# Kuldaen/Babylon.js-PathTracing-Renderer

Measured on AMD Instinct MI355X. Metric: Mpaths/s + achieved HBM GB/s, StanfordDragon 1080p 1spp, 1/2/4/8 MI355X, higher is better.
Workload: dtype f32

## Files before the change

### babylon.js-pathtracing-renderer_amd/csrc/pt_device.h

```cpp
#pragma once
#include <hip/hip_runtime.h>
#include <stdint.h>

#include "pt_args.h"
#include "pt_glsl.h"

namespace pt {
using namespace ptg;

constexpr float kINF = 1000000.0f;
constexpr float kTwoPi = 6.28318530717958648f;

enum { PROG_CORNELL = 3, PROG_GLTF = 4, PROG_HDRI = 5, PROG_SKY = 6, PROG_QUADRIC = 7, PROG_SKYMESH = 8 };
enum { PROG_TEX = 100, PROG_GLTF_TEX = 104, PROG_HDRI_TEX = 105, PROG_SKYMESH_TEX = 108 };
enum { PROG_PAIRS = 1000, PROG_TRAIL = 2000 };
template <int P> constexpr int kBase = P % PROG_PAIRS;
template <int P> constexpr int kScene = kBase<P> % PROG_TEX;
template <int P> constexpr bool kHasMesh = kScene<P> == PROG_GLTF || kScene<P> == PROG_HDRI || kScene<P> == PROG_SKYMESH;
template <int P> constexpr bool kIsGltf = kScene<P> == PROG_GLTF || kScene<P> == PROG_HDRI;
template <int P> constexpr bool kIsHdri = kScene<P> == PROG_HDRI;
template <int P> constexpr bool kHasTex = kBase<P> >= PROG_TEX;
template <int P> constexpr bool kIsSky = kScene<P> == PROG_SKY || kScene<P> == PROG_SKYMESH;
template <int P> constexpr bool kIsQuadric = P == PROG_QUADRIC;
template <int P> constexpr int kQuadId0 = kIsQuadric<P> ? 12 : 2;
template <int P> constexpr int kWalk = P / PROG_PAIRS;
template <int P> constexpr bool kPairs = P >= PROG_PAIRS;
template <int P> constexpr bool kTrail = kWalk<P> == WALK_TRAIL;
#define PT_FOR_EACH_PROG_REF(X)                                                                                           \
    X(PROG_CORNELL) X(PROG_SKY) X(PROG_QUADRIC) X(PROG_GLTF) X(PROG_GLTF_TEX) X(PROG_HDRI) X(PROG_HDRI_TEX)           \
    X(PROG_SKYMESH) X(PROG_SKYMESH_TEX)
#define PT_FOR_EACH_MESH_PROG(X, W)                                                                                       \
    X(W + PROG_GLTF) X(W + PROG_GLTF_TEX) X(W + PROG_HDRI) X(W + PROG_HDRI_TEX) X(W + PROG_SKYMESH) X(W + PROG_SKYMESH_TEX)
#define PT_FOR_EACH_PROG_PAIRS(X) PT_FOR_EACH_MESH_PROG(X, PROG_PAIRS)
#define PT_FOR_EACH_PROG_TRAIL(X) PT_FOR_EACH_MESH_PROG(X, PROG_TRAIL)
#define PT_FOR_EACH_PROG(X) PT_FOR_EACH_PROG_REF(X) PT_FOR_EACH_PROG_PAIRS(X) PT_FOR_EACH_PROG_TRAIL(X)

__host__ __device__ inline int resolveProgram(int prog, bool textured, int walk)
{
    if (prog != PROG_GLTF && prog != PROG_HDRI && prog != PROG_SKYMESH) return prog;
    return prog + (textured ? PROG_TEX : 0) + walk * PROG_PAIRS;
}
constexpr int kMinWavesTex = 4, kMinWavesPairs = 8, kMinWavesRef = 4;
template <int P> constexpr int kMinWaves = kHasTex<P> ? kMinWavesTex : kPairs<P> ? kMinWavesPairs : kMinWavesRef;
constexpr int kGoutLdsGltf = 0, kGoutLdsSky = 0;
template <int P> constexpr bool kPairs8 = kPairs<P> && !kHasTex<P>;
template <int P> constexpr int kGoutLdsOf = !kPairs8<P> ? 6 : kIsGltf<P> ? kGoutLdsGltf
                                          : kScene<P> == PROG_SKYMESH ? kGoutLdsSky : 6;
template <int P> constexpr int kStackLdsOf = kPairs8<P> ? (2 * kStackLdsPairs + 8 - kGoutLdsOf<P>) / 2 : kStackLds;
template <int P> constexpr int kRingOf = kHasTex<P> ? 14 : kPairs8<P> ? (2 * kStackLdsPairs + 8 - kGoutLdsOf<P>) / 2 : 6;
template <int P> constexpr bool kScratchOf = !kPairs8<P>;
template <int P> constexpr int kWalkSlotsOf = kTrail<P> ? kRingOf<P> : kStackLdsOf<P> + (kScratchOf<P> ? 1 : 0);

typedef float vf2 __attribute__((ext_vector_type(2)));
typedef __attribute__((address_space(3))) vf2 lds_float2;
typedef __attribute__((address_space(1))) vf2 glb_float2;

struct Path {
    uint32_t s0, s1;
    uint32_t bn;
    f3 ro, rd;
};
PT_D float unorm8(unsigned b);
PT_D float pathCounter(const Path& p) { return (float)((p.bn >> 16) & 0x7fu) - 1.0f; }
PT_D void setPathCounter(Path& p, float c) { p.bn = (p.bn & 0xff80ffffu) | ((unsigned)(c + 1.0f) << 16); }

PT_D float rng(Path& p)
{
    p.s0 += 1u; p.s1 += 1u;
    uint32_t qx = 1103515245u * ((p.s0 >> 1u) ^ p.s1);
    uint32_t qy = 1103515245u * ((p.s1 >> 1u) ^ p.s0);
    uint32_t n = 1103515245u * (qx ^ (qy >> 3u));
    return (float)n * (1.0f / 4294967296.0f);
}
PT_D float blueNoise_rand(Path& p)
{
    p.bn += 1u << 16;
    const unsigned channel = ((p.bn >> 16) - 1u) & 1u;
    return gfract(unorm8((p.bn >> (8u * channel)) & 255u));
}
PT_D float tentFilter(float x) { return (x < 0.5f) ? gsqrt(2.0f * x) - 1.0f : 1.0f - gsqrt(2.0f - (2.0f * x)); }
PT_D f3 onb_u(f3 nl)
{
    f3 a = (fabsf(nl.y) < 0.9f) ? mk(0.0f, 1.0f, 0.0f) : mk(1.0f, 0.0f, 0.0f);
    return normalize(cross(a, nl));
}
PT_D f3 cosWeightedDir(Path& p, f3 nl)
{
    float r = gsqrt(rng(p));
    float phi = rng(p) * kTwoPi;
    float sn, cs;
    gsincos(phi, sn, cs);
    float x = r * cs, y = r * sn;
    float z = gsqrt(1.0f - x * x - y * y);
    f3 U = onb_u(nl);
    f3 V = cross(nl, U);
    return normalize(U * x + V * y + nl * z);
}
PT_D f3 specularLobeDir(Path& p, f3 rdir, float roughness)
{
    roughness = gclamp(roughness, 0.0f, 1.0f);
    float exponent = gmix(7.0f, 0.0f, gsqrt(roughness));
    float cosTheta = gpow(rng(p), grcp(gexp(exponent) + 1.0f));
    float sinTheta = gsqrt(gmax(0.0f, 1.0f - cosTheta * cosTheta));
    float phi = rng(p) * kTwoPi;
    float sn, cs;
    gsincos(phi, sn, cs);
    f3 U = onb_u(rdir);
    f3 V = cross(rdir, U);
    f3 lobe = (U * cs) * sinTheta + (V * sn) * sinTheta + rdir * cosTheta;
    return normalize(mix3(rdir, lobe, roughness));
}
PT_D float fresnel(f3 rdir, f3 n, float etai, float etat, float& ratioIoR)
{
    float temp = etai;
    float cosi = gclamp(dot(rdir, n), -1.0f, 1.0f);
    if (cosi > 0.0f) { etai = etat; etat = temp; }
    ratioIoR = etai / etat;
    float sint = ratioIoR * gsqrt(1.0f - (cosi * cosi));
    if (sint >= 1.0f) return 1.0f;
    float cost = gsqrt(1.0f - (sint * sint));
    cosi = fabsf(cosi);
    float Rs = ((etat * cosi) - (etai * cost)) / ((etat * cosi) + (etai * cost));
    float Rp = ((etai * cosi) - (etat * cost)) / ((etai * cosi) + (etat * cost));
    return gclamp(((Rs * Rs) + (Rp * Rp)) * 0.5f, 0.0f, 1.0f);
}
PT_D f3 sampleQuadLight(Path& p, const TraceArgs& a, f3 x, f3 nl, float& weight)
{
    const QuadArg& L = a.light;
    f3 q;
    q.x = gmix(L.v0.x, L.v2.x, gclamp(rng(p), 0.1f, 0.9f));
    q.y = gmix(L.v0.y, L.v2.y, gclamp(rng(p), 0.1f, 0.9f));
    q.z = gmix(L.v0.z, L.v2.z, gclamp(rng(p), 0.1f, 0.9f));
    f3 d = q - x;
    float d2 = dot(d, d);
    float cos_a_max = gsqrt(1.0f - gclamp(a.light_r2 / d2, 0.0f, 1.0f));
    d = normalize(d);
    float dotNl = gmax(0.0f, dot(nl, d));
    float w = 2.0f * (1.0f - cos_a_max) * gmax(0.0f, -dot(d, L.normal)) * dotNl;
    weight = gclamp(w, 0.0f, 1.0f);
    return d;
}

PT_D float unitSphere(f3 ro, f3 rd, f3& n)
{
    float a = dot(rd, rd);
    float b = 2.0f * dot(rd, ro);
    float c = dot(ro, ro) - 1.0f;
    float invA = grcp(a);
    b *= invA;
    c *= invA;
    float nh = -b * 0.5f;
    float u2 = nh * nh - c;
    float u;
    if (u2 < 0.0f) { nh = 0.0f; u = 0.0f; } else u = gsqrt(u2);
    float t0 = nh - u, t1 = nh + u;
    float t = t0 > 0.0f ? t0 : t1 > 0.0f ? t1 : kINF;
    if (t != kINF) { f3 h = ro + rd * t; n = mk(2.0f * h.x, 2.0f * h.y, 2.0f * h.z); }
    return t;
}
PT_D bool recipNegative(float x) { return (x < 0.0f && x != -__builtin_inff()) || (x == 0.0f && __builtin_signbit(x)); }

PT_D float quadTriangle(const TriArg& T, f3 ro, f3 rd)
{
    f3 pv = cross(rd, T.e2);
    const float dd = dot(T.e1, pv);
    if (recipNegative(dd)) return kINF;
    float det = grcp(dd);
    f3 tv = ro - T.v0;
    float u = dot(tv, pv) * det;
    if (u < 0.0f || u > 1.0f) return kINF;
    f3 qv = cross(tv, T.e1);
    float v = dot(rd, qv) * det;
    float t = dot(T.e2, qv) * det;
    return (u < 0.0f || u > 1.0f || v < 0.0f || u + v > 1.0f || t <= 0.0f) ? kINF : t;
}
PT_D float box(f3 mn, f3 mx, f3 ro, f3 inv)
{
    f3 nr = (mn - ro) * inv;
    f3 fr = (mx - ro) * inv;
    float t0 = gmax(gmax(gmin(nr.x, fr.x), gmin(nr.y, fr.y)), gmin(nr.z, fr.z));
    float t1 = gmin(gmin(gmax(nr.x, fr.x), gmax(nr.y, fr.y)), gmax(nr.z, fr.z));
    return gmax(t0, 0.0f) > t1 ? kINF : t0;
}
PT_D float vmax0(float a) { float r; asm("v_max_f32 %0, 0, %1" : "=v"(r) : "v"(a)); return r; }
PT_D float boxFast(f3 mn, f3 mx, f3 ro, f3 inv)
{
    float t0, t1, a0, a1, a2, b0, b1, b2;
    asm("v_sub_f32 %2, %8, %14\n\t"
        "v_sub_f32 %3, %9, %15\n\t"
        "v_sub_f32 %4, %10, %16\n\t"
        "v_sub_f32 %5, %11, %14\n\t"
        "v_sub_f32 %6, %12, %15\n\t"
        "v_sub_f32 %7, %13, %16\n\t"
        "v_mul_f32 %2, %2, %17\n\t"
        "v_mul_f32 %3, %3, %18\n\t"
        "v_mul_f32 %4, %4, %19\n\t"
        "v_mul_f32 %5, %5, %17\n\t"
        "v_mul_f32 %6, %6, %18\n\t"
        "v_mul_f32 %7, %7, %19\n\t"
        "v_min_f32 %0, %2, %5\n\t"
        "v_max_f32 %2, %2, %5\n\t"
        "v_min_f32 %1, %3, %6\n\t"
        "v_max_f32 %3, %3, %6\n\t"
        "v_min_f32 %5, %4, %7\n\t"
// ... 394 lines not shown
```

### babylon.js-pathtracing-renderer_amd/csrc/pt_program.h

```cpp
#pragma once
#include <hip/hip_runtime.h>
#include <stdint.h>

#include "pt_args.h"
#include "pt_device.h"
#include "pt_glsl.h"
#include "pt_quadric.h"

namespace pt {

struct Hit {
    float t;
    f3 normal, color;
    float u, v;
    int type;
    int id;
};

struct Cnt {
    unsigned seg, node, leaf, hit, tap, ovf, hdr;
#ifdef PT_SECPROF
    unsigned long long* sec;
    unsigned lane_steps;
    unsigned sget, sget_slab, sput, sput_slab;
    unsigned bounce;
#endif
};
#ifdef PT_SECPROF
#define PT_SEC(cnt, k)                                                                        \
    do {                                                                                      \
        const unsigned long long now_ = clock64();                                            \
        const int ln_ = __lane_id();                                                          \
        if ((cnt).sec && ln_ == __builtin_amdgcn_readfirstlane(ln_)) {                \
            (cnt).sec[k] += now_ - (cnt).sec[8]; (cnt).sec[8] = now_;                         \
        }                                                                                     \
    } while (0)
#else
#define PT_SEC(cnt, k) do {} while (0)
#endif

struct GOut {
    static constexpr bool kColById = false;
    f3 nrm, col;
    float id, sharp;
    PT_D void clear() { nrm = mk(0, 0, 0); col = mk(0, 0, 0); id = 0.0f; sharp = 0.0f; }
    PT_D void pinCol(f3) {}
    PT_D void setNrm(f3 v) { nrm = v; }
    PT_D void setCol(f3 v) { col = v; }
    PT_D void setId(float v) { id = v; }
    PT_D void setSharp(float v) { sharp = v; }
};
typedef __attribute__((address_space(3))) float lds_float;
typedef __attribute__((address_space(1))) float glb_float;
template <int LS, int NF = 6>
struct GOutLds {
    static constexpr bool kColById = NF <= 3;
    lds_float* p;
    unsigned slot;
    glb_float* gx;
    unsigned gi, gs;
    uint32_t* bn;
    PT_D unsigned at(int f) const
    {
        unsigned i = gi;
        asm volatile("" : "+v"(i));
        return i + (unsigned)(f - NF) * gs;
    }
    PT_D void put(int f, float v)
    {
        if (f < NF) p[f * LS + slot] = v;
        else gx[at(f)] = v;
    }
    PT_D float get(int f) const
    {
        if (f < NF) return p[f * LS + slot];
        return ((*bn >> (f < 3 ? 23 : 31)) & 1u) ? gx[at(f)] : 0.0f;
    }
    PT_D void clear()
    {
        for (int f = 0; f < NF; f++) p[f * LS + slot] = 0.0f;
        *bn &= 0x007fffffu;
    }
    PT_D void setNrm(f3 v)
    {
        put(0, v.x); put(1, v.y); put(2, v.z);
        if (NF < 3 || kColById) *bn |= 1u << 23;
    }
    PT_D void setCol(f3 v)
    {
        if (kColById) return;
        put(3, v.x); put(4, v.y); put(5, v.z);
        if (NF < 6) *bn |= 1u << 31;
    }
    PT_D void pinCol(f3 v)
    {
        if (!kColById) return;
        put(3, v.x); put(4, v.y); put(5, v.z);
        *bn |= 1u << 31;
    }
    PT_D void setId(float v) { *bn = (*bn & ~(31u << 26)) | (((unsigned)(int)v & 31u) << 26); }
    PT_D void setSharp(float v)
    {
        const unsigned code = v == 1.01f ? 1u : v == -1.0f ? 2u : 0u;
        *bn = (*bn & ~(3u << 24)) | (code << 24);
    }
    PT_D float sharp() const
    {
        const unsigned code = (*bn >> 24) & 3u;
        return code == 1u ? 1.01f : code == 2u ? -1.0f : 0.0f;
    }
    PT_D float id() const { return (float)((*bn >> 26) & 31u); }
    template <class F>
    PT_D GOut load(F colOfId) const
    {
        GOut g;
        g.nrm = mk(get(0), get(1), get(2)); g.id = id(); g.sharp = sharp();
        if (!kColById) g.col = mk(get(3), get(4), get(5));
        else if (!((*bn >> 23) & 1u)) g.col = mk(0.0f, 0.0f, 0.0f);
        else g.col = ((*bn >> 31) & 1u) ? mk(get(3), get(4), get(5)) : colOfId(g.id);
        return g;
    }
};

struct PState {
    f3 mask;
    float roughness;
    int diffuseCount, hitType, bounce;
    bool coat, specular, sampleLight;
};

template <class G>
PT_D void pathBegin(PState& s, G& g)
{
    s.mask = mk(1, 1, 1);
    s.roughness = 0.0f;
    s.diffuseCount = 0; s.hitType = -100; s.bounce = 0;
    s.coat = false; s.specular = true; s.sampleLight = false;
    g.clear();
}

PT_D float rayleighPhase(float cosTheta) { return 0.05968310365946075f * (1.0f + (cosTheta * cosTheta)); }
PT_HD float hgPhase(float cosTheta, float g)
{
    float g2 = g * g;
    float inverse = grcp(gpow(gmax(0.0f, 1.0f - 2.0f * g * cosTheta + g2), 1.5f));
    return 0.07957747154594767f * ((1.0f - g2) * inverse);
}
PT_D f3 pow3(f3 v, float e) { return mk(gpow(v.x, e), gpow(v.y, e), gpow(v.z, e)); }
PT_D f3 skyColor(const SkyArgs& k, f3 rayDir)
{
    const f3 vd = normalize(rayDir);
    const float cosViewSunAngle = dot(vd, k.sun);
    const float zenithAngle = gacos(gmax(0.0f, dot(mk(0.0f, 1.0f, 0.0f), vd)));
    const float inverse =
        grcp(gcos(zenithAngle) + 0.15f * gpow(93.885f - ((zenithAngle * 180.0f) / 3.14159265358979323f), -1.253f));
    const float rl = 8400.0f * inverse, ml = 1250.0f * inverse;
    const f3 e = k.rayleigh * rl + k.mie * ml;
    const f3 Fex = mk(gexp(-e.x), gexp(-e.y), gexp(-e.z));
    const f3 betaR = k.rayleigh * rayleighPhase(cosViewSunAngle * 0.5f + 0.5f);
    const f3 betaM = k.mie * hgPhase(cosViewSunAngle, 0.76f);
    const f3 q = (betaR + betaM) / k.rm;
    f3 Lin = pow3((q * k.sunE) * (mk(1.0f, 1.0f, 1.0f) - Fex), 1.5f);
    const f3 m = pow3((q * k.sunE) * Fex, 1.0f / 2.0f);
    Lin = Lin * mk(gmix(1.0f, m.x, k.fade), gmix(1.0f, m.y, k.fade), gmix(1.0f, m.z, k.fade));
    f3 L0 = mk(0.1f, 0.1f, 0.1f) * Fex;
    const float sundisk = gsmoothstep(0.9998f, 0.9998f + 0.00002f, cosViewSunAngle);
    L0 = L0 + (Fex * k.sunE19000) * sundisk;
    const f3 tex = (Lin + L0) * 0.04f + mk(0.0f, 0.0003f, 0.00075f);
    return pow3(tex, k.retExp);
}

template <int PROG>
PT_D int meshObjectId(const TraceArgs& a) { return kQuadId0<PROG> + a.nquads; }

template <int PROG>
PT_D void objectMaterial(const TraceArgs& a, int id, f3& color, int& type)
{
    constexpr int q0 = kQuadId0<PROG>;
    if (kIsQuadric<PROG> && id >= 0 && id < q0) {
        const float cr[12] = { 1.0f, 0.0f, 1.0f, 1.0f, 1.0f, 0.5f, 0.0f, 0.0f, 0.2f, 0.0f, 1.0f, 0.5f };
        const float cg[12] = { 0.0f, 1.0f, 1.0f, 0.0f, 0.1f, 1.0f, 0.4f, 0.0f, 0.0f, 1.0f, 0.3f, 0.0f };
        const float cb[12] = { 0.0f, 0.0f, 0.0f, 1.0f, 0.0f, 0.0f, 1.0f, 1.0f, 1.0f, 0.5f, 0.0f, 1.0f };
        color = mk(cr[id], cg[id], cb[id]);
        type = a.shape_mat;
    } else if (!kIsQuadric<PROG> && id >= 0 && id < 2) {
        color = a.sph[id].color; type = a.sph[id].type;
    } else if (id >= q0 && id < q0 + a.nquads) {
        color = a.qcolor[id - q0]; type = a.qtype[id - q0];
    } else if (kHasMesh<PROG> && id == meshObjectId<PROG>(a)) {
        color = mk(1.0f, 1.0f, 1.0f); type = a.uses_albedo ? PBR_MATERIAL : a.model_mat;
    }
}

template <int PROG>
PT_D void analyticNearest(const TraceArgs& a, f3 rayO, f3 rayD, Hit& h, f3& sn)
{
    constexpr int q0 = kQuadId0<PROG>;
    h.t = kINF;
    h.type = -100;
    h.id = -1;
    sn = mk(0, 0, 0);
    if (kIsQuadric<PROG>) {
#pragma unroll 1
        for (int s = 0; s < 12; s++) {
            f3 n = mk(0, 0, 0);
            float d = quadricShape(s, mul(a.shape_inv[s], rayO, 1.0f), mul(a.shape_inv[s], rayD, 0.0f), a.shape_k, n);
            if (d < h.t) { h.t = d; h.id = s; sn = n; }
        }
    } else {
#pragma unroll 1
        for (int s = 0; s < 2; s++) {
            const SphereArg& S = a.sph[s];
            f3 n;
            float d = unitSphere(mul(S.inv, rayO, 1.0f), mul(S.inv, rayD, 0.0f), n);
            if (d < h.t) { h.t = d; h.id = s; sn = n; }
        }
    }
// ... 224 lines not shown
```

### babylon.js-pathtracing-renderer_amd/csrc/pt_trace.h

```cpp
#pragma once
#include <hip/hip_runtime.h>
#include <stdint.h>

#include "pt_args.h"
#include "pt_device.h"
#include "pt_glsl.h"
#include "pt_program.h"
#ifdef PT_SECPROF
#define PT_SECPROF_ON 1
#else
#define PT_SECPROF_ON 0
#endif

using namespace ptg;

namespace pt {

template <int LS, int NL, bool SCRATCH>
struct MegaStack {
    lds_float2* lds;
    unsigned slot;
    glb_float2* slab;
    unsigned deep;
    unsigned stride;
#ifdef PT_SECPROF
    mutable unsigned n_get = 0, n_get_slab = 0, n_put = 0, n_put_slab = 0;
#define PT_SLABCOUNT(x) x
#else
#define PT_SLABCOUNT(x)
#endif
    PT_D float2 pop(int si, float2 sentinel) const
    {
        PT_SLABCOUNT(n_get++; if (si >= NL) n_get_slab++;)
        vf2 e = lds[(unsigned)min(si, NL - 1) * LS + slot];
        if (si >= NL) {
            const vf2 s = { sentinel.x, sentinel.y };
            e = si < kStackLevels ? slab[(unsigned)(si - NL) * stride + deep] : s;
        }
        return make_float2(e.x, e.y);
    }
    PT_D bool push(int si, float2 e)
    {
        const vf2 v = { e.x, e.y };
        PT_SLABCOUNT(n_put++; if (si >= NL) n_put_slab++;)
        if (SCRATCH) lds[(unsigned)min(si, NL) * LS + slot] = v;
        else if (si < NL) lds[(unsigned)si * LS + slot] = v;
        if (si >= NL) {
            if (si >= kStackLevels) return false;
            slab[(unsigned)(si - NL) * stride + deep] = v;
        }
        return true;
    }
};

template <int PROG, bool COUNT>
PT_D void meshHit(const TraceArgs& a, float triID, float triU, float triV, Hit& h, Cnt& cnt)
{
    float4 v2 = fetch32(a.tri, a.tri_texels, triID + 2.0f), v3 = fetch32(a.tri, a.tri_texels, triID + 3.0f),
           v4 = fetch32(a.tri, a.tri_texels, triID + 4.0f), v5 = fetch32(a.tri, a.tri_texels, triID + 5.0f);
    if (COUNT) cnt.hit++;
    float triW = 1.0f - triU - triV;
    f3 nn = normalize(mk(v2.y, v2.z, v2.w) * triW + mk(v3.x, v3.y, v3.z) * triU + mk(v3.w, v4.x, v4.y) * triV);
    h.u = triW * v4.z + triU * v5.x + triV * v5.z;
    h.v = triW * v4.w + triU * v5.y + triV * v5.w;
    if (kHasTex<PROG> && a.uses_bump) {
        f3 S = onb_u(nn);
        f3 T = cross(nn, S);
        f3 N = normalize(nn);
        if (dot(cross(S, T), N) < 0.0f) { S = S * -1.0f; T = T * -1.0f; }
        float tx[4];
        texBilinear(a.bump, h.u, h.v, tx);
        if (COUNT) cnt.tap += 4;
        f3 mN = normalize(mk(tx[0] * 2.0f - 1.0f, tx[1] * 2.0f - 1.0f, tx[2] * 2.0f - 1.0f));
        mN.x *= 1.0f; mN.y *= 1.0f;
        nn = normalize(S * mN.x + T * mN.y + N * mN.z);
    }
    h.normal = normalize(mul3t(a.model, nn));
    h.type = a.uses_albedo ? PBR_MATERIAL : a.model_mat;
    h.color = mk(1.0f, 1.0f, 1.0f);
    h.id = meshObjectId<PROG>(a);
}

template <int PROG, bool COUNT, int LS>
PT_D void sceneIntersect(const TraceArgs& a, f3 rayO, f3 rayD, Hit& h, float2* lds, unsigned lane_slot,
                         unsigned deep, Cnt& cnt, bool firstHit)
{
    const bool anyHit = !COUNT && firstHit;
    if (COUNT) cnt.seg++;
    f3 sn;
    PT_SEC(cnt, 4);
    analyticNearest<PROG>(a, rayO, rayD, h, sn);
    PT_SEC(cnt, 1);
    if (!kHasMesh<PROG>) { analyticAttributes<PROG>(a, h, sn); PT_SEC(cnt, 3); return; }

    f3 O = mul(a.model, rayO, 1.0f), D = mul(a.model, rayD, 0.0f);
    f3 inv = mk(grcp(D.x), grcp(D.y), grcp(D.z));
    const bool dbl = (!a.uses_albedo && a.model_mat == TRANSPARENT);
    BvhResult br = { 0.0f, 0.0f, 0.0f, false, 1u, 0u, 0u };
    MegaStack<LS, kStackLdsOf<PROG>, kScratchOf<PROG>> st{ (lds_float2*)lds, lane_slot, (glb_float2*)a.spill, deep, a.spill_stride };
    if (kPairs<PROG>) {
        const float* rb = a.bvh_root_box;
        const float rootT = box(mk(rb[0], rb[1], rb[2]), mk(rb[3], rb[4], rb[5]), O, inv);
        auto walk = [&]() {
            if (kTrail<PROG>) bvhWalkTrail<kRingOf<PROG>>(a, O, D, inv, dbl, rootT, h.t, (lds_float2*)lds, LS, lane_slot, br);
            else bvhWalkPairs(a, O, D, inv, dbl, rootT, h.t, st, br, anyHit);
        };
#ifdef PT_SECPROF
        if (cnt.sec) {
            const int ln_ = __lane_id();
            if (ln_ == __builtin_amdgcn_readfirstlane(ln_)) cnt.sec[9] = 0;
            walk();
            atomicMax(&cnt.sec[9], (unsigned long long)br.steps);
            cnt.lane_steps += br.steps;
            if (ln_ == __builtin_amdgcn_readfirstlane(ln_)) cnt.sec[10] += cnt.sec[9];
        } else
#endif
        walk();
    } else {
        float4 c0 = fetch32(a.aabb, a.aabb_texels, 0.0f), c1 = fetch32(a.aabb, a.aabb_texels, 1.0f);
        const float rootT = box(mk(c0.y, c0.z, c0.w), mk(c1.y, c1.z, c1.w), O, inv);
        bvhWalkRef(a, O, D, inv, dbl, c0, c1, rootT, h.t, st, br);
    }
    if (COUNT) { cnt.node += br.nodes; cnt.leaf += br.leaves; cnt.ovf += br.ovf; }
#ifdef PT_SECPROF
    if (COUNT) { cnt.sget += st.n_get; cnt.sget_slab += st.n_get_slab + br.restarts; cnt.sput += st.n_put; cnt.sput_slab += st.n_put_slab; }
    br.ws.flush(a.walk_stat, cnt.bounce++);
#endif
    PT_SEC(cnt, 2);
    if (br.lookup && anyHit) {
        h.normal = mk(0.0f, 0.0f, 1.0f);
        h.type = a.uses_albedo ? PBR_MATERIAL : a.model_mat;
        h.color = mk(1.0f, 1.0f, 1.0f);
        h.id = meshObjectId<PROG>(a);
    } else if (br.lookup) meshHit<PROG, COUNT>(a, br.triID, br.triU, br.triV, h, cnt);
    else analyticAttributes<PROG>(a, h, sn);
    PT_SEC(cnt, 3);
}

template <int PROG, bool COUNT, int LS, class G>
PT_D bool bounceStep(const TraceArgs& a, Path& p, PState& s, G& g, f3& accum, float2* lds, unsigned lane_slot,
                     unsigned deep, Cnt& cnt)
{
    Hit h;
    const bool lastOk = !kHasTex<PROG> && !a.uses_albedo &&
                        (a.model_mat == DIFFUSE || a.model_mat == METAL || a.model_mat == TRANSPARENT);
    sceneIntersect<PROG, COUNT, LS>(a, p.ro, p.rd, h, lds, lane_slot, deep, cnt, s.sampleLight || (s.bounce == 5 && lastOk));
    return shadeStep<PROG, COUNT, G>(a, p, s, g, accum, h, cnt);
}

PT_D void contStore(const TraceArgs& a, unsigned slot, const Path& p, const PState& s)
{
    const unsigned bits = ((unsigned)s.diffuseCount & 0xffu) | (((unsigned)s.hitType & 0xffu) << 8) |
                          (((unsigned)s.bounce & 0xffu) << 16) | (s.coat ? 1u << 24 : 0u) |
                          (s.specular ? 1u << 25 : 0u) | (s.sampleLight ? 1u << 26 : 0u);
    float4* r = a.cont_rec + 4ull * slot;
    r[0] = make_float4(p.ro.x, p.ro.y, p.ro.z, p.rd.x);
    r[1] = make_float4(p.rd.y, p.rd.z, s.mask.x, s.mask.y);
    r[2] = make_float4(s.mask.z, s.roughness, __uint_as_float(p.s0), __uint_as_float(p.s1));
    r[3] = make_float4(__uint_as_float(p.bn), __uint_as_float(bits), 0.0f, 0.0f);
}
PT_D void contLoad(const TraceArgs& a, unsigned slot, Path& p, PState& s)
{
    const float4* r = a.cont_rec + 4ull * slot;
    const float4 r0 = r[0], r1 = r[1], r2 = r[2], r3 = r[3];
    p.ro = mk(r0.x, r0.y, r0.z); p.rd = mk(r0.w, r1.x, r1.y);
    s.mask = mk(r1.z, r1.w, r2.x); s.roughness = r2.y;
    p.s0 = __float_as_uint(r2.z); p.s1 = __float_as_uint(r2.w); p.bn = __float_as_uint(r3.x);
    const unsigned bits = __float_as_uint(r3.y);
    s.diffuseCount = (int)(bits & 0xffu);
    s.hitType = (int)(signed char)((bits >> 8) & 0xffu);
    s.bounce = (int)((bits >> 16) & 0xffu);
    s.coat = (bits >> 24) & 1u; s.specular = (bits >> 25) & 1u; s.sampleLight = (bits >> 26) & 1u;
}
struct GBits {
    static constexpr bool kColById = false;
    uint32_t* bn;
    PT_D void clear() {}
    PT_D void pinCol(f3) {}
    PT_D void setNrm(f3) {}
    PT_D void setCol(f3) {}
    PT_D void setId(float) {}
    PT_D float id() const { return 0.0f; }
    PT_D void setSharp(float v)
    {
        const unsigned code = v == 1.01f ? 1u : v == -1.0f ? 2u : 0u;
        *bn = (*bn & ~(3u << 24)) | (code << 24);
    }
    PT_D float sharp() const
    {
        const unsigned code = (*bn >> 24) & 3u;
        return code == 1u ? 1.01f : code == 2u ? -1.0f : 0.0f;
    }
};

PT_D void contRank(const TraceArgs& a, int slot, const Path& p, const PState& s, bool inside)
{
    unsigned key = 0u;
    if (inside) {
        const float* rb = a.bvh_root_box;
        const f3 o = mul(a.model, p.ro, 1.0f);
        const unsigned gb = a.cont_grid_bits;
        const int top = (1 << gb) - 1;
        const unsigned cx = (unsigned)min(top, max(0, (int)((o.x - rb[0]) * a.cont_cell[0])));
        const unsigned cy = (unsigned)min(top, max(0, (int)((o.y - rb[1]) * a.cont_cell[1])));
        const unsigned cz = (unsigned)min(top, max(0, (int)((o.z - rb[2]) * a.cont_cell[2])));
        auto spread = [](unsigned v) { return (v & 1u) | ((v & 2u) << 2) | ((v & 4u) << 4); };
        const unsigned cell = spread(cx) | (spread(cy) << 1) | (spread(cz) << 2);
        const unsigned oct = (p.rd.x < 0.0f ? 1u : 0u) | (p.rd.y < 0.0f ? 2u : 0u) | (p.rd.z < 0.0f ? 4u : 0u);
        const unsigned lt = s.sampleLight ? 1u : 0u;
        key = (lt << (3u + 3u * gb)) | (cell << 3) | oct;
    }
    unsigned long long todo = __ballot(inside), peers = 0ull;
    while (todo) {
        const int lead = __ffsll((long long)todo) - 1;
        const unsigned k = __shfl(key, lead, 64);
        const bool mine = inside && key == k;
        const unsigned long long m = __ballot(mine);
        if (mine) peers = m;
        todo &= ~m;
    }
    const int leader = inside ? __ffsll((long long)peers) - 1 : (int)__lane_id();
    unsigned base = 0u;
    if (inside && (int)__lane_id() == leader) base = atomicAdd(&a.cont_bins[key], (unsigned)__popcll(peers));
    base = __shfl(base, leader, 64);
    if (inside) {
        a.cont_key[slot] = (unsigned short)key;
        a.cont_rank[slot] = base + (unsigned)__popcll(peers & ((1ull << __lane_id()) - 1ull));
    }
}

template <int PROG, bool COUNT, int LS, bool CONT, class G>
PT_D f3 radiance(const TraceArgs& a, Path& p, G& g, float2* lds, unsigned lane_slot, unsigned deep, Cnt& cnt,
                 bool inside, int& slot)
{
    PState s;
    pathBegin(s, g);
    f3 accum = mk(0, 0, 0);
#pragma unroll 1
    while (bounceStep<PROG, COUNT, LS, G>(a, p, s, g, accum, lds, lane_slot, deep, cnt)) {
        if (CONT && (unsigned)s.bounce >= a.cont_bounce && (unsigned)__popcll(__ballot(1)) <= a.cont_lanes) {
            const unsigned long long st = __ballot(inside);
            const int lead = __ffsll((long long)__ballot(1)) - 1;
            unsigned base = 0;
            if (__lane_id() == lead && st) base = atomicAdd(a.cont_count, (unsigned)__popcll(st));
            base = __shfl(base, lead, 64);
            if (inside) {
                slot = (int)(base + (unsigned)__popcll(st & ((1ull << __lane_id()) - 1ull)));
                contStore(a, (unsigned)slot, p, s);
            }
            if (a.cont_bins) contRank(a, slot, p, s, inside);
            break;
        }
    }
    return max3s(accum, 0.0f);
}

PT_D void radianceOut(const TraceArgs& a, long long pi, f3 r, float sharp, bool edge)
{
    float ca = 0.0f;
    if (edge) sharp = 1.01f;
    if (sharp == 1.01f) ca = 1.01f;
    if (sharp == -1.0f) ca = -1.0f;
    typedef float nt4 __attribute__((ext_vector_type(4)));
    const nt4 o = { r.x, r.y, r.z, ca };
    __builtin_nontemporal_store(o, (nt4*)&a.rad[pi]);
}

PT_D void featureOut(const TraceArgs& a, long long pi, const GOut& g)
{
    typedef float nt4 __attribute__((ext_vector_type(4)));
    const nt4 n = { g.nrm.x, g.nrm.y, g.nrm.z, g.id };
    const nt4 c = { g.col.x, g.col.y, g.col.z, 0.0f };
    __builtin_nontemporal_store(n, (nt4*)&a.feat0[pi]);
    __builtin_nontemporal_store(c, (nt4*)&a.feat1[pi]);
}

PT_D float xorq(float v, int m) { return __shfl_xor(v, m, 64); }

constexpr int kCostBuckets = 128;

constexpr int kTraceBlock = 64;
constexpr int kTraceSub = 4;

struct TracePlace {
    int px, py, part;
    unsigned costIdx;
};
PT_D bool tracePlace(const TraceArgs& a, int lane, TracePlace& pl)
{
    int wave, part = -1;
    const unsigned tiles_x = gridDim.x / 4u, ntiles = a.ntiles;
    const unsigned K = (a.order && a.split) ? *a.split : 0u;
    const unsigned L = blockIdx.y * gridDim.x + blockIdx.x;
    unsigned slot;
    constexpr unsigned kPer = 4u * kSplitParts;
    if (L < kPer * K) {
        const unsigned g = L / (8u * kPer), r = L % (8u * kPer);
        slot = g * 8u + (r & 7u);
        wave = (int)((r >> 3) / kSplitParts);
        part = (int)((r >> 3) % kSplitParts);
    } else {
        const unsigned L2 = L - kPer * K;
        if (L2 >= 4u * (ntiles - K)) return false;
        const unsigned g = L2 >> 5, r = L2 & 31u;
        const unsigned T = min(8u, ntiles - K - g * 8u);
        slot = K + g * 8u + r % T;
        wave = (int)(r / T);
    }
    unsigned rank = slot;
    if (a.order_zig && slot >= K) {
        const unsigned j = slot - K, m = ntiles - K, g = j >> 3, t = (g >> 1) * 8u + (j & 7u);
        rank = K + ((g & 1u) ? m - 1u - t : t);
    }
    const unsigned tile = a.order ? a.order[rank] : slot;
    const int tx = (int)(tile % tiles_x);
    const unsigned bY = tile / tiles_x;
    int lx, ly;
    if (part < 0) { lx = (lane & 1) | ((lane >> 1) & 6); ly = ((lane >> 1) & 1) | ((lane >> 3) & 6); }
    else {
        lx = (part & 1) * 4 + ((lane & 1) | ((lane >> 1) & 2));
        ly = (part >> 1) * 4 + (((lane >> 1) & 1) | ((lane >> 2) & 2));
    }
    const int band = (int)bY * a.num_parts + a.part;
    pl.px = tx * kTile + (wave & 1) * 8 + lx;
    pl.py = band * kTile + (wave >> 1) * 8 + ly;
    pl.part = part;
    pl.costIdx = tile * 4u + (unsigned)wave;
    return true;
}

template <int PROG, bool COUNT, bool CONT, bool FEAT = false>
__global__ __launch_bounds__(kTraceBlock, kMinWaves<PROG>) void pt_trace(TraceArgs a)
{
    static_assert(!CONT || (kHasMesh<PROG> && !COUNT), "late-bounce compaction: mesh programs, timed kernels");
    static_assert(!FEAT || !COUNT, "feature staging: a variant of the timed kernels");
    __shared__ float2 lds_stack[kWalkSlotsOf<PROG> * kTraceBlock + (kGoutLdsOf<PROG> * kTraceBlock + 1) / 2];
    float* const lds_gout = (float*)(lds_stack + kWalkSlotsOf<PROG> * kTraceBlock);
    const unsigned tid = threadIdx.x;
    const int lane = tid & 63;
    const unsigned long long t_start = clock64();
#ifdef PT_SECPROF
    const unsigned long long w0_ = wall_clock64();
#endif
    TracePlace pl;
    if (!tracePlace(a, lane, pl)) return;
    const int px = pl.px, py = pl.py;
    const unsigned deep = (blockIdx.y * gridDim.x + blockIdx.x) * kTraceBlock + tid;

    const bool active = px < ((a.width + 1) & ~1) && py < ((a.height + 1) & ~1) && (pl.part < 0 || lane < (int)(64u / kSplitParts));
    Cnt cnt = { 0, 0, 0, 0, 0, 0, 0 };
#ifdef PT_SECPROF
    __shared__ unsigned long long lds_sec[16];
    if (tid < 16) lds_sec[tid] = tid == 8 ? clock64() : 0ull;
    cnt.sec = lds_sec;
    cnt.lane_steps = 0;
    cnt.sget = cnt.sget_slab = cnt.sput = cnt.sput_slab = 0;
    cnt.bounce = 0;
#endif
    glb_float* const gx = kGoutLdsOf<PROG> < 6
        ? (glb_float*)(a.spill + (size_t)(kStackLevels - kStackLdsMin) * a.spill_stride)
        : nullptr;
    Path p;
    p.bn = 0u;
    GOutLds<kTraceBlock, kGoutLdsOf<PROG>> gl{ (lds_float*)lds_gout, tid, gx, deep, a.spill_stride, &p.bn };
    gl.clear();
    f3 r = mk(0, 0, 0);
    int slot = -1;
    if (active) {
        cameraRay(a, px, py, p);
        PT_SEC(cnt, 0);
        r = radiance<PROG, COUNT, kTraceBlock, CONT>(a, p, gl, lds_stack, tid, deep, cnt, px < a.width && py < a.height, slot);
    }
    PT_SEC(cnt, 4);
    const GOut g = gl.load([&](float id) {
        f3 c = mk(0.0f, 0.0f, 0.0f);
        int t;
        objectMaterial<PROG>(a, (int)id, c, t);
        return c;
    });

    const bool xodd = lane & 1, yodd = lane & 2;
    auto ddx = [&](float v) { float o = xorq(v, 1); return xodd ? v - o : o - v; };
    auto ddy = [&](float v) { float o = xorq(v, 2); return yodd ? v - o : o - v; };
    float dNx = fabsf(ddx(g.nrm.x)) + fabsf(ddy(g.nrm.x));
    float dNy = fabsf(ddx(g.nrm.y)) + fabsf(ddy(g.nrm.y));
    float dNz = fabsf(ddx(g.nrm.z)) + fabsf(ddy(g.nrm.z));
    float normalDiff = gsmoothstep(0.2f, 0.6f, dNx) + gsmoothstep(0.2f, 0.6f, dNy) + gsmoothstep(0.2f, 0.6f, dNz);
    float dObj = fabsf(ddx(g.id)) > 0.0f ? 1.0f : 0.0f;
    dObj += fabsf(ddy(g.id)) > 0.0f ? 1.0f : 0.0f;
    float objectDiff = gsmoothstep(0.0f, 0.5f, dObj);
    f3 dcx = mk(ddx(g.col.x), ddx(g.col.y), ddx(g.col.z));
    f3 dcy = mk(ddy(g.col.x), ddy(g.col.y), ddy(g.col.z));
    float dCol = length(dcx) > 0.0f ? 1.0f : 0.0f;
    dCol += length(dcy) > 0.0f ? 1.0f : 0.0f;
    float colorDiff = gsmoothstep(0.0f, 0.5f, dCol);

#ifdef PT_SECPROF
    if (!COUNT && a.wave_log) {
        atomicMax(&lds_sec[11], (unsigned long long)cnt.lane_steps);
        if (tid == 0) {
            const unsigned L = blockIdx.y * gridDim.x + blockIdx.x;
            unsigned long long* wl = a.wave_log + (size_t)kWaveLogSlots * L;
            wl[0] = w0_;
            wl[1] = wall_clock64();
            wl[2] = lds_sec[10];
            wl[3] = lds_sec[11];
            for (int k = 0; k < 8; k++) wl[4 + k] = lds_sec[k];
            wl[12] = __smid();
        }
    }
    if (COUNT && active) {
        atomicAdd(&a.counters[3], (unsigned long long)cnt.sget_slab);
        atomicAdd(&a.counters[4], (unsigned long long)cnt.node);
        atomicAdd(&a.counters[5], (unsigned long long)cnt.leaf);
        atomicAdd(&a.counters[6], 1ull);
    }
#endif
    if (COUNT && active && !PT_SECPROF_ON) {
        unsigned long long* C = a.counters;
        atomicAdd(&C[C_PATHS], 1ull);
        atomicAdd(&C[C_SEGMENTS], (unsigned long long)cnt.seg);
        atomicAdd(&C[C_NODE], (unsigned long long)cnt.node);
        atomicAdd(&C[C_LEAF], (unsigned long long)cnt.leaf);
        atomicAdd(&C[C_HIT], (unsigned long long)cnt.hit);
        atomicAdd(&C[C_RGBA8], (unsigned long long)(cnt.tap + 1));
        atomicAdd(&C[C_OVERFLOW], (unsigned long long)cnt.ovf);
        atomicAdd(&C[C_HDR], (unsigned long long)cnt.hdr);
    }
    if (a.cost && lane == 0) {
        const unsigned long long dur = min(clock64() - t_start, 0xffffffffull);
        a.cost[pl.costIdx] = (unsigned)((dur + (unsigned long long)a.cost[pl.costIdx]) >> 1);
    }
    if (!active || px >= a.width || py >= a.height) return;
    const bool edge = colorDiff >= 1.0f || normalDiff >= 1.0f || objectDiff >= 1.0f;
    const long long pi = (long long)py * a.width + px;
    if (FEAT || (COUNT && a.feat0)) featureOut(a, pi, g);
    if (CONT && slot >= 0) {
        a.cont_aux[slot] = (unsigned)pi | (edge ? 0x80000000u : 0u);
        return;
    }
    radianceOut(a, pi, r, g.sharp, edge);
}

template <int PROG>
__global__ __launch_bounds__(kTraceBlock, kMinWaves<PROG>) void pt_cont(TraceArgs a)
{
    __shared__ float2 lds_stack[kWalkSlotsOf<PROG> * kTraceBlock];
    const unsigned lane = threadIdx.x;
    const unsigned n = a.cont_count[0];
    unsigned* const head = a.cont_count + 1;
    bool more = true;
    const unsigned deep = blockIdx.x * kTraceBlock + lane;
    const unsigned long long below = (1ull << lane) - 1ull;
    Cnt cnt = { 0, 0, 0, 0, 0, 0, 0 };
    Path p;
    p.bn = 0u;
    PState s;
    GBits g{ &p.bn };
    f3 accum = mk(0, 0, 0);
    unsigned slot = 0;
    bool alive = false;
    for (;;) {
        const unsigned long long dead = __ballot(!alive);
        const unsigned ndead = (unsigned)__popcll(dead);
        if (more && (ndead >= a.cont_refill || ndead == 64u)) {
            unsigned base = 0;
            if (lane == 0) base = atomicAdd(head, ndead);
            base = __shfl(base, 0, 64);
            if (base + ndead >= n) more = false;
            if (!alive) {
                const unsigned q = base + (unsigned)__popcll(dead & below);
                if (q < n) {
                    slot = a.cont_perm ? a.cont_perm[q] : q;
                    contLoad(a, slot, p, s);
                    accum = mk(0, 0, 0);
                    alive = true;
                }
            }
        }
        if (__ballot(alive) == 0ull) {
            if (!more) break;
            continue;
        }
        if (alive && !bounceStep<PROG, false, kTraceBlock>(a, p, s, g, accum, lds_stack, lane, deep, cnt)) {
            const unsigned aux = a.cont_aux[slot];
            radianceOut(a, (long long)(aux & 0x7fffffffu), max3s(accum, 0.0f), g.sharp(), (aux >> 31) != 0u);
            alive = false;
        }
    }
}

template <int PROG, bool COUNT>
__global__ __launch_bounds__(kBlock, kMinWaves<PROG>) void pt_persist(TraceArgs a, WfBufs w, int tiles_x,
                                                                       unsigned n_wave_tiles, unsigned per_wave,
                                                                       unsigned refill)
{
    __shared__ float2 lds_stack[kWalkSlotsOf<PROG> * kBlock];
    const unsigned tid = threadIdx.x;
    const unsigned lane = tid & 63u, wave = tid >> 6;
    const unsigned long long below = (1ull << lane) - 1ull;
    const unsigned wid = blockIdx.x * (kBlock / 64) + wave;
    unsigned next = wid * per_wave * 64u;
    const unsigned end = min(next + per_wave * 64u, n_wave_tiles * 64u);
    const unsigned deep = blockIdx.x * kBlock + tid;
    Cnt cnt = { 0, 0, 0, 0, 0, 0, 0 };
    unsigned paths = 0;
    Path p;
    PState s;
    GOut g;
    f3 accum = mk(0, 0, 0);
    unsigned pix = 0;
    bool alive = false;
    for (;;) {
        const unsigned long long dead = __ballot(!alive);
        const unsigned ndead = (unsigned)__popcll(dead);
        if (next < end && (ndead >= refill || ndead == 64u)) {
            if (!alive) {
                const unsigned q = next + (unsigned)__popcll(dead & below);
                if (q < end) {
                    const unsigned L = q >> 6, l = q & 63u;
                    const unsigned per_band = (unsigned)tiles_x * 4u;
                    const unsigned bl = L / per_band, rem = L - bl * per_band;
                    const unsigned tx = rem >> 2, sub = rem & 3u;
                    const int band = (int)bl * a.num_parts + a.part;
                    const int lx = (int)((l & 1u) | ((l >> 1) & 6u)), ly = (int)(((l >> 1) & 1u) | ((l >> 3) & 6u));
                    const int px = (int)tx * kTile + (int)(sub & 1u) * 8 + lx;
                    const int py = band * kTile + (int)(sub >> 1) * 8 + ly;
                    if (px < w.wq && py < w.hq) {
                        cameraRay(a, px, py, p);
                        pathBegin(s, g);
                        accum = mk(0, 0, 0);
                        pix = (unsigned)py * (unsigned)w.wq + (unsigned)px;
                        alive = true;
                        if (COUNT) paths++;
                    }
                }
            }
            next += ndead;
        }
        if (__ballot(alive) == 0ull) {
            if (next >= end) break;
            continue;
        }
        if (alive && !bounceStep<PROG, COUNT, kBlock>(a, p, s, g, accum, lds_stack, tid, deep, cnt)) {
            const f3 r = max3s(accum, 0.0f);
            w.gb0[pix] = make_float4(g.nrm.x, g.nrm.y, g.nrm.z, g.id);
            w.gb1[pix] = make_float4(g.col.x, g.col.y, g.col.z, g.sharp);
            w.rad[pix] = make_float4(r.x, r.y, r.z, 0.0f);
            alive = false;
        }
    }
    if (COUNT) {
        unsigned long long* C = a.counters;
        if (paths) atomicAdd(&C[C_PATHS], (unsigned long long)paths);
        atomicAdd(&C[C_SEGMENTS], (unsigned long long)cnt.seg);
        atomicAdd(&C[C_NODE], (unsigned long long)cnt.node);
        atomicAdd(&C[C_LEAF], (unsigned long long)cnt.leaf);
        atomicAdd(&C[C_HIT], (unsigned long long)cnt.hit);
        atomicAdd(&C[C_RGBA8], (unsigned long long)(cnt.tap + paths));
        atomicAdd(&C[C_OVERFLOW], (unsigned long long)cnt.ovf);
        atomicAdd(&C[C_HDR], (unsigned long long)cnt.hdr);
    }
}

}
```

Measured before the change: 3225.

## Recompute lane-derived indices and pack path state to cut live VGPRs across traversal

For the pairs BVH programs, the kernel stops keeping per-lane values live through BVH traversal. Spill and gout addresses now use a wave-uniform base plus the lane id recomputed with mbcnt. Pixel coordinates and the inside test are rebuilt after tracing, path state flags are packed into one register across sceneIntersect, and the sphere normal is recomputed after traversal. The continuation kernel keeps only mask, roughness and packed bits between steps. The aim is lower register pressure and higher occupancy in the traversal loop, at the cost of extra ALU work to recompute and unpack these values.

```diff
diff --git a/babylon.js-pathtracing-renderer_amd/csrc/pt_device.h b/babylon.js-pathtracing-renderer_amd/csrc/pt_device.h
--- a/babylon.js-pathtracing-renderer_amd/csrc/pt_device.h
+++ b/babylon.js-pathtracing-renderer_amd/csrc/pt_device.h
@@ -50,6 +50,14 @@
 template <int P> constexpr int kRingOf = kHasTex<P> ? 14 : kPairs8<P> ? (2 * kStackLdsPairs + 8 - kGoutLdsOf<P>) / 2 : 6;
 template <int P> constexpr bool kScratchOf = !kPairs8<P>;
 template <int P> constexpr int kWalkSlotsOf = kTrail<P> ? kRingOf<P> : kStackLdsOf<P> + (kScratchOf<P> ? 1 : 0);
+
+template <int P> constexpr bool kWaveBaseOf = kPairs8<P>;
+PT_D unsigned laneNow()
+{
+    unsigned l;
+    asm volatile("v_mbcnt_lo_u32_b32 %0, -1, 0\n\tv_mbcnt_hi_u32_b32 %0, -1, %0" : "=v"(l));
+    return l;
+}
 
 typedef float vf2 __attribute__((ext_vector_type(2)));
 typedef __attribute__((address_space(3))) vf2 lds_float2;
diff --git a/babylon.js-pathtracing-renderer_amd/csrc/pt_pathstate.h b/babylon.js-pathtracing-renderer_amd/csrc/pt_pathstate.h
--- /dev/null
+++ b/babylon.js-pathtracing-renderer_amd/csrc/pt_pathstate.h
@@ -0,0 +1,22 @@
+#pragma once
+#include <cstdint>
+
+namespace pt {
+
+struct PathBits {
+    int diffuseCount, hitType, bounce;
+    bool coat, specular, sampleLight;
+};
+
+constexpr uint32_t pathBitsPack(int diffuseCount, int hitType, int bounce, bool coat, bool specular, bool sampleLight)
+{
+    return ((uint32_t)diffuseCount & 0xffu) | (((uint32_t)hitType & 0xffu) << 8) | (((uint32_t)bounce & 0xffu) << 16) |
+           (coat ? 1u << 24 : 0u) | (specular ? 1u << 25 : 0u) | (sampleLight ? 1u << 26 : 0u);
+}
+constexpr PathBits pathBitsUnpack(uint32_t bits)
+{
+    return PathBits{ (int)(bits & 0xffu), (int)(((bits >> 8) & 0xffu) ^ 0x80u) - 0x80, (int)((bits >> 16) & 0xffu),
+                     ((bits >> 24) & 1u) != 0u, ((bits >> 25) & 1u) != 0u, ((bits >> 26) & 1u) != 0u };
+}
+
+}
diff --git a/babylon.js-pathtracing-renderer_amd/csrc/pt_program.h b/babylon.js-pathtracing-renderer_amd/csrc/pt_program.h
--- a/babylon.js-pathtracing-renderer_amd/csrc/pt_program.h
+++ b/babylon.js-pathtracing-renderer_amd/csrc/pt_program.h
@@ -52,7 +52,7 @@
 };
 typedef __attribute__((address_space(3))) float lds_float;
 typedef __attribute__((address_space(1))) float glb_float;
-template <int LS, int NF = 6>
+template <int LS, int NF = 6, bool BASE = false>
 struct GOutLds {
     static constexpr bool kColById = NF <= 3;
     lds_float* p;
@@ -62,7 +62,7 @@
     uint32_t* bn;
     PT_D unsigned at(int f) const
     {
-        unsigned i = gi;
+        unsigned i = BASE ? gi + laneNow() : gi;
         asm volatile("" : "+v"(i));
         return i + (unsigned)(f - NF) * gs;
     }
diff --git a/babylon.js-pathtracing-renderer_amd/csrc/pt_trace.h b/babylon.js-pathtracing-renderer_amd/csrc/pt_trace.h
--- a/babylon.js-pathtracing-renderer_amd/csrc/pt_trace.h
+++ b/babylon.js-pathtracing-renderer_amd/csrc/pt_trace.h
@@ -5,6 +5,7 @@
 #include "pt_args.h"
 #include "pt_device.h"
 #include "pt_glsl.h"
+#include "pt_pathstate.h"
 #include "pt_program.h"
 #ifdef PT_SECPROF
 #define PT_SECPROF_ON 1
@@ -16,13 +17,14 @@
 
 namespace pt {
 
-template <int LS, int NL, bool SCRATCH>
+template <int LS, int NL, bool SCRATCH, bool BASE>
 struct MegaStack {
     lds_float2* lds;
     unsigned slot;
     glb_float2* slab;
     unsigned deep;
     unsigned stride;
+    PT_D unsigned at() const { return BASE ? deep + laneNow() : deep; }
 #ifdef PT_SECPROF
     mutable unsigned n_get = 0, n_get_slab = 0, n_put = 0, n_put_slab = 0;
 #define PT_SLABCOUNT(x) x
@@ -35,7 +37,7 @@
         vf2 e = lds[(unsigned)min(si, NL - 1) * LS + slot];
         if (si >= NL) {
             const vf2 s = { sentinel.x, sentinel.y };
-            e = si < kStackLevels ? slab[(unsigned)(si - NL) * stride + deep] : s;
+            e = si < kStackLevels ? slab[(unsigned)(si - NL) * stride + at()] : s;
         }
         return make_float2(e.x, e.y);
     }
@@ -47,7 +49,7 @@
         else if (si < NL) lds[(unsigned)si * LS + slot] = v;
         if (si >= NL) {
             if (si >= kStackLevels) return false;
-            slab[(unsigned)(si - NL) * stride + deep] = v;
+            slab[(unsigned)(si - NL) * stride + at()] = v;
         }
         return true;
     }
@@ -81,7 +83,22 @@
     h.id = meshObjectId<PROG>(a);
 }
 
-template <int PROG, bool COUNT, int LS>
+template <int PROG> constexpr bool kNormalAfter = kHasMesh<PROG> && !kIsQuadric<PROG>;
+PT_D f3 sphereNormal(const TraceArgs& a, f3 rayO, f3 rayD, const Hit& h)
+{
+    f3 n = mk(0, 0, 0);
+#pragma unroll 1
+    for (int s = 0; s < 2; s++) {
+        if (h.id != s) continue;
+        const SphereArg& S = a.sph[s];
+        const f3 ro = mul(S.inv, rayO, 1.0f), rd = mul(S.inv, rayD, 0.0f);
+        const f3 x = ro + rd * h.t;
+        n = mk(2.0f * x.x, 2.0f * x.y, 2.0f * x.z);
+    }
+    return n;
+}
+
+template <int PROG, bool COUNT, int LS, bool SLIM>
 PT_D void sceneIntersect(const TraceArgs& a, f3 rayO, f3 rayD, Hit& h, float2* lds, unsigned lane_slot,
                          unsigned deep, Cnt& cnt, bool firstHit)
 {
@@ -97,7 +114,7 @@
     f3 inv = mk(grcp(D.x), grcp(D.y), grcp(D.z));
     const bool dbl = (!a.uses_albedo && a.model_mat == TRANSPARENT);
     BvhResult br = { 0.0f, 0.0f, 0.0f, false, 1u, 0u, 0u };
-    MegaStack<LS, kStackLdsOf<PROG>, kScratchOf<PROG>> st{ (lds_float2*)lds, lane_slot, (glb_float2*)a.spill, deep, a.spill_stride };
+    MegaStack<LS, kStackLdsOf<PROG>, kScratchOf<PROG>, SLIM> st{ (lds_float2*)lds, lane_slot, (glb_float2*)a.spill, deep, a.spill_stride };
     if (kPairs<PROG>) {
         const float* rb = a.bvh_root_box;
         const float rootT = box(mk(rb[0], rb[1], rb[2]), mk(rb[3], rb[4], rb[5]), O, inv);
@@ -133,44 +150,56 @@
         h.color = mk(1.0f, 1.0f, 1.0f);
         h.id = meshObjectId<PROG>(a);
     } else if (br.lookup) meshHit<PROG, COUNT>(a, br.triID, br.triU, br.triV, h, cnt);
-    else analyticAttributes<PROG>(a, h, sn);
+    else {
+        if (SLIM && kNormalAfter<PROG>) sn = sphereNormal(a, rayO, rayD, h);
+        analyticAttributes<PROG>(a, h, sn);
+    }
     PT_SEC(cnt, 3);
 }
 
-template <int PROG, bool COUNT, int LS, class G>
+PT_D unsigned pathBitsOf(const PState& s)
+{
+    return pathBitsPack(s.diffuseCount, s.hitType, s.bounce, s.coat, s.specular, s.sampleLight);
+}
+PT_D void pathBitsTo(PState& s, unsigned bits)
+{
+    const PathBits b = pathBitsUnpack(bits);
+    s.diffuseCount = b.diffuseCount; s.hitType = b.hitType; s.bounce = b.bounce;
+    s.coat = b.coat; s.specular = b.specular; s.sampleLight = b.sampleLight;
+}
+
+template <int PROG, bool COUNT, int LS, bool SLIM, class G>
 PT_D bool bounceStep(const TraceArgs& a, Path& p, PState& s, G& g, f3& accum, float2* lds, unsigned lane_slot,
                      unsigned deep, Cnt& cnt)
 {
     Hit h;
     const bool lastOk = !kHasTex<PROG> && !a.uses_albedo &&
                         (a.model_mat == DIFFUSE || a.model_mat == METAL || a.model_mat == TRANSPARENT);
-    sceneIntersect<PROG, COUNT, LS>(a, p.ro, p.rd, h, lds, lane_slot, deep, cnt, s.sampleLight || (s.bounce == 5 && lastOk));
+    const bool firstHit = s.sampleLight || (s.bounce == 5 && lastOk);
+    unsigned bits = pathBitsOf(s);
+    if (SLIM) asm volatile("" : "+v"(bits));
+    sceneIntersect<PROG, COUNT, LS, SLIM>(a, p.ro, p.rd, h, lds, lane_slot, deep, cnt, firstHit);
+    if (SLIM) { asm volatile("" : "+v"(bits)); pathBitsTo(s, bits); }
     return shadeStep<PROG, COUNT, G>(a, p, s, g, accum, h, cnt);
 }
 
 PT_D void contStore(const TraceArgs& a, unsigned slot, const Path& p, const PState& s)
 {
-    const unsigned bits = ((unsigned)s.diffuseCount & 0xffu) | (((unsigned)s.hitType & 0xffu) << 8) |
-                          (((unsigned)s.bounce & 0xffu) << 16) | (s.coat ? 1u << 24 : 0u) |
-                          (s.specular ? 1u << 25 : 0u) | (s.sampleLight ? 1u << 26 : 0u);
+    const unsigned bits = pathBitsOf(s);
     float4* r = a.cont_rec + 4ull * slot;
     r[0] = make_float4(p.ro.x, p.ro.y, p.ro.z, p.rd.x);
     r[1] = make_float4(p.rd.y, p.rd.z, s.mask.x, s.mask.y);
     r[2] = make_float4(s.mask.z, s.roughness, __uint_as_float(p.s0), __uint_as_float(p.s1));
     r[3] = make_float4(__uint_as_float(p.bn), __uint_as_float(bits), 0.0f, 0.0f);
 }
-PT_D void contLoad(const TraceArgs& a, unsigned slot, Path& p, PState& s)
+PT_D void contLoad(const TraceArgs& a, unsigned slot, Path& p, f3& mask, float& roughness, unsigned& bits)
 {
     const float4* r = a.cont_rec + 4ull * slot;
     const float4 r0 = r[0], r1 = r[1], r2 = r[2], r3 = r[3];
     p.ro = mk(r0.x, r0.y, r0.z); p.rd = mk(r0.w, r1.x, r1.y);
-    s.mask = mk(r1.z, r1.w, r2.x); s.roughness = r2.y;
+    mask = mk(r1.z, r1.w, r2.x); roughness = r2.y;
     p.s0 = __float_as_uint(r2.z); p.s1 = __float_as_uint(r2.w); p.bn = __float_as_uint(r3.x);
-    const unsigned bits = __float_as_uint(r3.y);
-    s.diffuseCount = (int)(bits & 0xffu);
-    s.hitType = (int)(signed char)((bits >> 8) & 0xffu);
-    s.bounce = (int)((bits >> 16) & 0xffu);
-    s.coat = (bits >> 24) & 1u; s.specular = (bits >> 25) & 1u; s.sampleLight = (bits >> 26) & 1u;
+    bits = __float_as_uint(r3.y);
 }
 struct GBits {
     static constexpr bool kColById = false;
@@ -229,16 +258,17 @@
     }
 }
 
-template <int PROG, bool COUNT, int LS, bool CONT, class G>
+template <int PROG, bool COUNT, int LS, bool CONT, class G, class IN>
 PT_D f3 radiance(const TraceArgs& a, Path& p, G& g, float2* lds, unsigned lane_slot, unsigned deep, Cnt& cnt,
-                 bool inside, int& slot)
+                 IN insideNow, int& slot)
 {
     PState s;
     pathBegin(s, g);
     f3 accum = mk(0, 0, 0);
 #pragma unroll 1
-    while (bounceStep<PROG, COUNT, LS, G>(a, p, s, g, accum, lds, lane_slot, deep, cnt)) {
+    while (bounceStep<PROG, COUNT, LS, kWaveBaseOf<PROG>, G>(a, p, s, g, accum, lds, lane_slot, deep, cnt)) {
         if (CONT && (unsigned)s.bounce >= a.cont_bounce && (unsigned)__popcll(__ballot(1)) <= a.cont_lanes) {
+            const bool inside = insideNow();
             const unsigned long long st = __ballot(inside);
             const int lead = __ffsll((long long)__ballot(1)) - 1;
             unsigned base = 0;
@@ -275,6 +305,11 @@
     __builtin_nontemporal_store(c, (nt4*)&a.feat1[pi]);
 }
 
+PT_D unsigned lanesBelow(unsigned long long mask)
+{
+    return __builtin_amdgcn_mbcnt_hi((unsigned)(mask >> 32), __builtin_amdgcn_mbcnt_lo((unsigned)mask, 0u));
+}
+
 PT_D float xorq(float v, int m) { return __shfl_xor(v, m, 64); }
 
 constexpr int kCostBuckets = 128;
@@ -285,7 +320,16 @@
 struct TracePlace {
     int px, py, part;
     unsigned costIdx;
+    int x0, y0;
 };
+PT_D void placeLane(int part, int lane, int& lx, int& ly)
+{
+    if (part < 0) { lx = (lane & 1) | ((lane >> 1) & 6); ly = ((lane >> 1) & 1) | ((lane >> 3) & 6); }
+    else {
+        lx = (part & 1) * 4 + ((lane & 1) | ((lane >> 1) & 2));
+        ly = (part >> 1) * 4 + (((lane >> 1) & 1) | ((lane >> 2) & 2));
+    }
+}
 PT_D bool tracePlace(const TraceArgs& a, int lane, TracePlace& pl)
 {
     int wave, part = -1;
@@ -316,14 +360,12 @@
     const int tx = (int)(tile % tiles_x);
     const unsigned bY = tile / tiles_x;
     int lx, ly;
-    if (part < 0) { lx = (lane & 1) | ((lane >> 1) & 6); ly = ((lane >> 1) & 1) | ((lane >> 3) & 6); }
-    else {
-        lx = (part & 1) * 4 + ((lane & 1) | ((lane >> 1) & 2));
-        ly = (part >> 1) * 4 + (((lane >> 1) & 1) | ((lane >> 2) & 2));
-    }
+    placeLane(part, lane, lx, ly);
     const int band = (int)bY * a.num_parts + a.part;
-    pl.px = tx * kTile + (wave & 1) * 8 + lx;
-    pl.py = band * kTile + (wave >> 1) * 8 + ly;
+    pl.x0 = tx * kTile + (wave & 1) * 8;
+    pl.y0 = band * kTile + (wave >> 1) * 8;
+    pl.px = pl.x0 + lx;
+    pl.py = pl.y0 + ly;
     pl.part = part;
     pl.costIdx = tile * 4u + (unsigned)wave;
     return true;
@@ -337,17 +379,25 @@
     __shared__ float2 lds_stack[kWalkSlotsOf<PROG> * kTraceBlock + (kGoutLdsOf<PROG> * kTraceBlock + 1) / 2];
     float* const lds_gout = (float*)(lds_stack + kWalkSlotsOf<PROG> * kTraceBlock);
     const unsigned tid = threadIdx.x;
-    const int lane = tid & 63;
+    int lane = tid & 63;
     const unsigned long long t_start = clock64();
 #ifdef PT_SECPROF
     const unsigned long long w0_ = wall_clock64();
 #endif
     TracePlace pl;
     if (!tracePlace(a, lane, pl)) return;
-    const int px = pl.px, py = pl.py;
-    const unsigned deep = (blockIdx.y * gridDim.x + blockIdx.x) * kTraceBlock + tid;
-
-    const bool active = px < ((a.width + 1) & ~1) && py < ((a.height + 1) & ~1) && (pl.part < 0 || lane < (int)(64u / kSplitParts));
+    int px = pl.px, py = pl.py;
+    constexpr bool kWaveBase = kWaveBaseOf<PROG>;
+    if (kWaveBase) {
+        pl.x0 = __builtin_amdgcn_readfirstlane(pl.x0); pl.y0 = __builtin_amdgcn_readfirstlane(pl.y0);
+        pl.part = __builtin_amdgcn_readfirstlane(pl.part); pl.costIdx = __builtin_amdgcn_readfirstlane(pl.costIdx);
+    }
+    const unsigned deep = (blockIdx.y * gridDim.x + blockIdx.x) * kTraceBlock + (kWaveBase ? 0u : tid);
+
+    auto activeAt = [&](int x, int y, int ln) {
+        return x < ((a.width + 1) & ~1) && y < ((a.height + 1) & ~1) && (pl.part < 0 || ln < (int)(64u / kSplitParts));
+    };
+    bool active = activeAt(px, py, lane);
     Cnt cnt = { 0, 0, 0, 0, 0, 0, 0 };
 #ifdef PT_SECPROF
     __shared__ unsigned long long lds_sec[16];
@@ -362,14 +412,28 @@
         : nullptr;
     Path p;
     p.bn = 0u;
-    GOutLds<kTraceBlock, kGoutLdsOf<PROG>> gl{ (lds_float*)lds_gout, tid, gx, deep, a.spill_stride, &p.bn };
+    GOutLds<kTraceBlock, kGoutLdsOf<PROG>, kWaveBase> gl{ (lds_float*)lds_gout, tid, gx, deep, a.spill_stride, &p.bn };
     gl.clear();
     f3 r = mk(0, 0, 0);
     int slot = -1;
     if (active) {
         cameraRay(a, px, py, p);
         PT_SEC(cnt, 0);
-        r = radiance<PROG, COUNT, kTraceBlock, CONT>(a, p, gl, lds_stack, tid, deep, cnt, px < a.width && py < a.height, slot);
+        const bool inside0 = px < a.width && py < a.height;
+        auto insideNow = [&]() {
+            if (!kWaveBase) return inside0;
+            int lx, ly;
+            placeLane(pl.part, (int)laneNow(), lx, ly);
+            return pl.x0 + lx < a.width && pl.y0 + ly < a.height;
+        };
+        r = radiance<PROG, COUNT, kTraceBlock, CONT>(a, p, gl, lds_stack, tid, deep, cnt, insideNow, slot);
+    }
+    if (kWaveBase) {
+        lane = (int)laneNow();
+        int lx, ly;
+        placeLane(pl.part, lane, lx, ly);
+        px = pl.x0 + lx; py = pl.y0 + ly;
+        active = activeAt(px, py, lane);
     }
     PT_SEC(cnt, 4);
     const GOut g = gl.load([&](float id) {
@@ -450,14 +514,14 @@
     const unsigned n = a.cont_count[0];
     unsigned* const head = a.cont_count + 1;
     bool more = true;
-    const unsigned deep = blockIdx.x * kTraceBlock + lane;
-    const unsigned long long below = (1ull << lane) - 1ull;
+    const unsigned deep = blockIdx.x * kTraceBlock + (kWaveBaseOf<PROG> ? 0u : lane);
     Cnt cnt = { 0, 0, 0, 0, 0, 0, 0 };
     Path p;
     p.bn = 0u;
-    PState s;
+    f3 mask = mk(0, 0, 0);
+    float roughness = 0.0f;
+    unsigned bits = 0u;
     GBits g{ &p.bn };
-    f3 accum = mk(0, 0, 0);
     unsigned slot = 0;
     bool alive = false;
     for (;;) {
@@ -466,14 +530,13 @@
         if (more && (ndead >= a.cont_refill || ndead == 64u)) {
             unsigned base = 0;
             if (lane == 0) base = atomicAdd(head, ndead);
-            base = __shfl(base, 0, 64);
+            base = __builtin_amdgcn_readfirstlane(base);
             if (base + ndead >= n) more = false;
             if (!alive) {
-                const unsigned q = base + (unsigned)__popcll(dead & below);
+                const unsigned q = base + lanesBelow(dead);
                 if (q < n) {
                     slot = a.cont_perm ? a.cont_perm[q] : q;
-                    contLoad(a, slot, p, s);
-                    accum = mk(0, 0, 0);
+                    contLoad(a, slot, p, mask, roughness, bits);
                     alive = true;
                 }
             }
@@ -482,10 +545,21 @@
             if (!more) break;
             continue;
         }
-        if (alive && !bounceStep<PROG, false, kTraceBlock>(a, p, s, g, accum, lds_stack, lane, deep, cnt)) {
-            const unsigned aux = a.cont_aux[slot];
-            radianceOut(a, (long long)(aux & 0x7fffffffu), max3s(accum, 0.0f), g.sharp(), (aux >> 31) != 0u);
-            alive = false;
+        f3 accum = mk(0, 0, 0);
+        if (alive) {
+            PState s;
+            s.mask = mask;
+            s.roughness = kHasTex<PROG> ? roughness : 0.0f;
+            pathBitsTo(s, bits);
+            const bool go = bounceStep<PROG, false, kTraceBlock, kWaveBaseOf<PROG>>(a, p, s, g, accum, lds_stack, lane, deep, cnt);
+            mask = s.mask; roughness = s.roughness;
+            bits = pathBitsOf(s);
+            if (kWaveBaseOf<PROG>) asm volatile("" : "+v"(bits));
+            if (!go) {
+                const unsigned aux = a.cont_aux[slot];
+                radianceOut(a, (long long)(aux & 0x7fffffffu), max3s(accum, 0.0f), g.sharp(), (aux >> 31) != 0u);
+                alive = false;
+            }
         }
     }
 }
@@ -542,7 +616,7 @@
             if (next >= end) break;
             continue;
         }
-        if (alive && !bounceStep<PROG, COUNT, kBlock>(a, p, s, g, accum, lds_stack, tid, deep, cnt)) {
+        if (alive && !bounceStep<PROG, COUNT, kBlock, false>(a, p, s, g, accum, lds_stack, tid, deep, cnt)) {
             const f3 r = max3s(accum, 0.0f);
             w.gb0[pix] = make_float4(g.nrm.x, g.nrm.y, g.nrm.z, g.id);
             w.gb1[pix] = make_float4(g.col.x, g.col.y, g.col.z, g.sharp);
```

Result: faster. 3486, median of 6 (+8.1%).
